# google/neural-light-transport

Hardware: AMD Instinct MI355X
Metric: rendered Mtexels/s at 1024^2 UV (full Model.call forward: U-Net + UV->camera warp); at N > 1: N collective-free replicas of this forward (weak scaling).  The data-parallel TRAIN step with the RCCL gradient all-reduce (BASELINE config 4) is `train_step`: value = Mtexels/s over all ranks, speedup_vs_o (higher is better)
Workload: dtype f32 via 3xbf16 split, 9 exact products, fp32 accumulate (the LDS-tiled encoder convs: fp32 operands as three bf16 terms on v_mfma_f32_16x16x32_bf16, every term product exact in fp32); f32 storage everywhere, every other launch native f32; 1 GPU; BASELINE config 3: dragon_specular relight+view-synth, depth0 16/depth 256, 4 frames/GPU, 1024^2 UV, k=4 obs maps, 512^2 camera warp; frames_per_gpu=4, uv=1024, k=4, cam=512, conv_algo=auto, plan=fused ends, launch=eager, two HIP streams, distinct_batches_rotated=3, launch_tape_replays=0, parallelism=dp1 (frames sharded, no forward collective), world=1, dist_world_size=1, device=cuda:0

## Files before the change

include/nlt_hip.h:

```cpp
#ifndef NLT_HIP_H_
#define NLT_HIP_H_

#ifdef __cplusplus
extern "C" {
#endif

typedef enum {
  NLT_OK = 0,
  NLT_ERR_BAD_ARG = -1,
  NLT_ERR_UNSUPPORTED = -2,
  NLT_ERR_LAUNCH = -3
} nlt_status;

typedef enum {
  NLT_CONV1X1 = 0,
  NLT_CONV_K2S2 = 1,
  NLT_CONV_K2S1 = 2,
  NLT_DECONV_K2S2 = 3,
  NLT_DECONV_K2S1 = 4,
  NLT_CONV_K3S1 = 5,
  NLT_CONV_K3S2 = 6,
  NLT_DECONV_K3S1 = 7,
  NLT_DECONV_K3S2 = 8
} nlt_conv_mode;
// ... 399 lines not shown
                                const float* packed, int cout, int tn, float* out, int ldo,
                                const float* mask_src, int ldm, float mask_alpha, int accumulate, void* stream);

int nlt_conv_c32_supported(int mode, int cin, int cout);
int nlt_conv_c32_forward(int mode, const float* src, int ld, int cin, int frames, int kobs, int h, int w,
                         const float* packed, const float* bias, int cout,
                         float* out, int ldo, float* mean_out, int ldm, int act, float alpha, void* stream);

long nlt_conv_tile_packed_floats(int mode, int cin, int cout, int tn);
int nlt_pack_conv_tile_weights(int mode, const float* w_keras, int cin, int cout, int tn, float* packed, void* stream);
int nlt_conv_tile_forward(int mode, const float* src, int ld, int cin, int frames, int kobs, int h, int w,
                          const float* packed, const float* bias, int cout, int tn,
                          float* out, int ldo, float* mean_out, int ldm, int act, float alpha, void* stream);

int nlt_pack_conv_tile_weights_adjoint(int adj_mode, const float* w_keras, int cpre, int cout, int tn, int full, int lo,
                                       float* packed, void* stream);
int nlt_conv_tile_backward_data(int adj_mode, const float* dpre, int ldp, int cpre, int n, int h, int w,
                                const float* packed, int cout, int tn, float* out, int ldo,
                                const float* mask_src, int ldm, float mask_alpha, int accumulate,
                                int split_c, const float* split_y, float* split_d, float split_alpha, int split_partial,
                                void* stream);

long nlt_conv_tile3_packed_elems(int mode, int cin, int cout, int tn);
int nlt_pack_conv_tile3_weights(int mode, const float* w_keras, int cin, int cout, int tn, unsigned short* packed, void* stream);
int nlt_conv_tile3_forward(int mode, int nprod, const float* src, int ld, int cin, int frames, int kobs, int h, int w,
                           const unsigned short* packed, const float* bias, int cout, int tn,
                           float* out, int ldo, float* mean_out, int ldm, int act, float alpha, void* stream);
int nlt_conv_tile3r_forward(int mode, int nprod, const float* src, int ld, int cin, int frames, int kobs, int h, int w,
                            const unsigned short* packed, const float* bias, int cout, int tn,
                            float* out, int ldo, float* mean_out, int ldm, int act, float alpha, int max_workgroups, void* stream);
int nlt_conv_tile3d_forward(int mode, int nprod, const float* src, int ld, int cin, int frames, int kobs, int h, int w,
                            const unsigned short* packed, const float* bias, int cout, int tn,
                            float* out, int ldo, float* mean_out, int ldm, int act, float alpha, void* stream);
long nlt_conv_tile3w_s2_packed_elems(int cin2, int cout2);
int nlt_pack_conv_tile3w_s2_weights(const float* w_keras, int cin2, int cout2, unsigned short* packed, void* stream);
long nlt_conv_tile3w_s2_lds_bytes(int cin, int cout, int cout2);
int nlt_conv_tile3w_s2_forward(int nprod, const float* src, int ld, int cin, int frames, int kobs, int h, int w,
                               const unsigned short* packed, const float* bias, int cout, float* out, int ldo,
                               float* mean_out, int ldm, int act, float alpha,
                               const unsigned short* packed2, const float* bias2, int cout2, float* out2, int ldo2,
                               int act2, float alpha2, int max_workgroups, void* stream);

long nlt_chmix_bf16_packed_elems(int cin, int cout);
int nlt_chmix_bf16_pack(const float* w_keras, int cin, int cout, unsigned short* packed, void* stream);
int nlt_chmix_bf16_forward(const unsigned short* x, long texels, int cin, const unsigned short* packed,
                           const float* bias, int cout, int act, float alpha, unsigned short* out, void* stream);

int nlt_conv_k3_forward(int mode, int algo, const float* x, int n, int h, int w, int cin,
                        const float* w_keras, const float* bias, int cout, float* y,
                        int act, float alpha, void* stream);

int nlt_conv_k3_backward_data(int mode, int algo, const float* dpre, int n, int h, int w, int cin,
                              const float* w_keras, int cout, float* dx, void* stream);

long nlt_conv_k3_wgrad_workspace_floats(int mode, int n, int h, int w, int cin, int cout);
int nlt_conv_k3_backward_weights(int mode, const float* x, int n, int h, int w, int cin,
                                 const float* dpre, int cout, float* dw_keras, float* dbias,
                                 float* workspace, long workspace_floats, void* stream);

#ifdef __cplusplus
}
#endif
#endif
```

neural-light-transport_amd/_capi.py:

```python
import ctypes
import threading
import os

import torch

_HERE = os.path.dirname(os.path.abspath(__file__))
LIB_PATH = os.environ.get('NLT_HIP_LIB') or os.path.join(_HERE, 'libnlt_hip.so')

CONV1X1, CONV_K2S2, CONV_K2S1, DECONV_K2S2, DECONV_K2S1 = range(5)
CONV_K3S1, CONV_K3S2, DECONV_K3S1, DECONV_K3S2 = range(5, 9)
ALGO_AUTO, ALGO_DIRECT, ALGO_MFMA = range(3)

_c_int, _c_long, _c_float, _vp = ctypes.c_int, ctypes.c_long, ctypes.c_float, ctypes.c_void_p
_c_double = ctypes.c_double
MAP_F64, MAP_F32, MAP_F16 = range(3)

SIGNATURES = {
    'nlt_version': (ctypes.c_char_p, []),
    'nlt_status_string': (ctypes.c_char_p, [_c_int]),
    'nlt_packed_weight_floats': (_c_long, [_c_int] * 4),
    'nlt_pack_conv_weights': (_c_int, [_c_int, _vp, _c_int, _c_int, _c_int, _vp, _vp]),
    'nlt_conv_forward': (_c_int, [_c_int, _c_int, _c_int, _vp, _c_int, _c_int, _vp, _c_int, _c_int,
                                  _c_int, _c_int, _c_int, _vp, _vp, _vp, _c_int, _vp, _c_int,
                                  _c_int, _c_float, _vp, _c_int, _c_int, _vp]),
# ... 83 lines not shown
    'nlt_front_ovr_forward_u8': (_c_int, [_vp] * 4 + [_c_int] * 3 + [_vp] * 5 + [_c_int, _c_float, _vp, _c_int, _vp, _vp, _vp]),
    'nlt_front_obs_forward': (_c_int, [_vp, _vp] + [_c_int] * 3 + [_vp, _vp, _c_float, _c_int] + [_vp] * 3 + [_vp]),
    'nlt_front_obs_forward_u8': (_c_int, [_vp] * 3 + [_c_int] * 3 + [_vp, _vp, _c_float, _c_int] + [_vp] * 3 + [_vp]),
    'nlt_frame_sum_accumulate': (_c_int, [_vp, _c_int, _c_long, _vp, _c_int, _vp]),
    'nlt_frame_mean_finish': (_c_int, [_vp, _c_long, _c_long, _vp, _vp]),
    'nlt_frame_mean_finish_l0': (_c_int, [_vp, _c_long, _c_long, _vp, _vp, _vp, _vp]),
    'nlt_conv_backward_data': (_c_int, [_c_int, _c_int, _c_int, _vp, _vp, _c_int, _c_int, _c_int, _c_int, _c_int, _vp, _vp, _c_int,
                                        _vp, _c_int, _vp, _c_int, _c_float, _c_int, _c_int, _vp, _vp, _c_float, _c_int, _vp]),
    'nlt_conv_tile_packed_floats': (_c_long, [_c_int] * 4),
    'nlt_pack_conv_tile_weights': (_c_int, [_c_int, _vp, _c_int, _c_int, _c_int, _vp, _vp]),
    'nlt_conv_tile_forward': (_c_int, [_c_int, _vp, _c_int, _c_int, _c_int, _c_int, _c_int, _c_int, _vp, _vp, _c_int, _c_int,
                                       _vp, _c_int, _vp, _c_int, _c_int, _c_float, _vp]),
    'nlt_pack_conv_tile_weights_adjoint': (_c_int, [_c_int, _vp, _c_int, _c_int, _c_int, _c_int, _c_int, _vp, _vp]),
    'nlt_conv_c32_supported': (_c_int, [_c_int] * 3),
    'nlt_conv_c32_forward': (_c_int, [_c_int, _vp, _c_int, _c_int, _c_int, _c_int, _c_int, _c_int, _vp, _vp, _c_int,
                                      _vp, _c_int, _vp, _c_int, _c_int, _c_float, _vp]),
    'nlt_conv_wino_packed_floats': (_c_long, [_c_int] * 4),
    'nlt_pack_conv_wino_weights': (_c_int, [_c_int, _vp, _c_int, _c_int, _c_int, _vp, _vp]),
    'nlt_conv_wino_forward': (_c_int, [_c_int, _vp, _c_int, _c_int, _c_int, _c_int, _c_int, _c_int, _vp, _vp, _c_int, _c_int,
                                       _vp, _c_int, _vp, _c_int, _c_int, _c_float, _vp]),
    'nlt_pack_conv_wino_weights_adjoint': (_c_int, [_c_int, _vp, _c_int, _c_int, _c_int, _c_int, _c_int, _vp, _vp]),
    'nlt_conv_wino_backward_data': (_c_int, [_c_int, _vp, _c_int, _c_int, _c_int, _c_int, _c_int, _vp, _c_int, _c_int, _vp, _c_int,
                                             _vp, _c_int, _c_float, _c_int, _vp]),
    'nlt_conv_tile_backward_data': (_c_int, [_c_int, _vp, _c_int, _c_int, _c_int, _c_int, _c_int, _vp, _c_int, _c_int, _vp, _c_int,
                                             _vp, _c_int, _c_float, _c_int, _c_int, _vp, _vp, _c_float, _c_int, _vp]),
    'nlt_conv_tile3_packed_elems': (_c_long, [_c_int] * 4),
    'nlt_pack_conv_tile3_weights': (_c_int, [_c_int, _vp, _c_int, _c_int, _c_int, _vp, _vp]),
    'nlt_conv_tile3_forward': (_c_int, [_c_int, _c_int, _vp, _c_int, _c_int, _c_int, _c_int, _c_int, _c_int, _vp, _vp, _c_int, _c_int,
                                        _vp, _c_int, _vp, _c_int, _c_int, _c_float, _vp]),
    'nlt_conv_tile3r_forward': (_c_int, [_c_int, _c_int, _vp, _c_int, _c_int, _c_int, _c_int, _c_int, _c_int, _vp, _vp, _c_int, _c_int,
                                         _vp, _c_int, _vp, _c_int, _c_int, _c_float, _c_int, _vp]),
    'nlt_conv_tile3d_forward': (_c_int, [_c_int, _c_int, _vp, _c_int, _c_int, _c_int, _c_int, _c_int, _c_int, _vp, _vp, _c_int, _c_int,
                                         _vp, _c_int, _vp, _c_int, _c_int, _c_float, _vp]),
    'nlt_conv_tile3w_s2_packed_elems': (_c_long, [_c_int] * 2),
    'nlt_pack_conv_tile3w_s2_weights': (_c_int, [_vp, _c_int, _c_int, _vp, _vp]),
    'nlt_conv_tile3w_s2_lds_bytes': (_c_long, [_c_int] * 3),
    'nlt_conv_tile3w_s2_forward': (_c_int, [_c_int, _vp, _c_int, _c_int, _c_int, _c_int, _c_int, _c_int, _vp, _vp, _c_int, _vp, _c_int,
                                            _vp, _c_int, _c_int, _c_float, _vp, _vp, _c_int, _vp, _c_int, _c_int, _c_float, _c_int, _vp]),
    'nlt_conv_bf16_packed_elems': (_c_long, [_c_int] * 4),
    'nlt_conv_bf16_pack': (_c_int, [_c_int, _vp, _c_int, _c_int, _c_int, _vp, _vp]),
    'nlt_conv_bf16_forward': (_c_int, [_c_int, _c_int, _vp, _c_int, _c_int, _c_int, _vp, _c_int, _c_int, _c_int,
                                       _c_int, _c_int, _c_int, _vp, _vp, _c_int, _vp, _c_int, _c_int, _c_int, _c_float, _vp]),
    'nlt_conv_bf16_forward_map': (_c_int, [_c_int, _c_int, _vp, _c_int, _c_int, _c_int, _vp, _c_int, _c_int, _c_int,
                                           _c_int, _c_int, _c_int, _vp, _vp, _c_int, _vp, _c_int, _c_int, _c_int, _c_float,
                                           _vp, _c_int, _vp]),
    'nlt_obs_mean_bf16': (_c_int, [_vp, _c_int, _c_int, _c_long, _c_int, _vp, _c_int, _vp]),
    'nlt_chmix_bf16_packed_elems': (_c_long, [_c_int, _c_int]),
    'nlt_chmix_bf16_pack': (_c_int, [_vp, _c_int, _c_int, _vp, _vp]),
    'nlt_chmix_bf16_forward': (_c_int, [_vp, _c_long, _c_int, _vp, _vp, _c_int, _c_int, _c_float, _vp, _vp]),
    'nlt_cosine_map': (_c_int, [_vp] * 4 + [_c_double] * 3 + [_c_long, _vp, _vp, _vp]),
    'nlt_albedo': (_c_int, [_vp, _c_int, _c_long, _vp, _vp, _vp]),
    'nlt_diffuse_base': (_c_int, [_vp, _vp, _c_int, _c_long, _vp, _vp]),
    'nlt_remap_bilinear_u8': (_c_int, [_vp, _c_int, _c_int, _c_int, _vp, _c_int, _c_int, _c_int, _c_int, _c_int, _vp, _vp]),
    'nlt_remap_bilinear_f32': (_c_int, [_vp, _c_int, _c_int, _c_int, _vp, _c_int, _c_int, _c_int, _c_int, _c_int, _vp, _vp]),
    'nlt_capture_camspc': (_c_int, [_vp] * 4 + [_c_double] * 6 + [_vp, _vp, _c_int, _c_int] + [_vp] * 5),
    'nlt_capture_uvspc': (_c_int, [_vp, _c_int, _c_int, _c_int, _vp, _vp, _vp, _c_int, _c_int, _c_int] + [_vp] * 6),
    'nlt_diffuse_bases': (_c_int, [_vp, _vp, _vp] + [_c_int] * 5 + [_vp, _vp, _vp]),
    'nlt_uv_index_map_workspace_bytes': (_c_long, [_c_int, _c_int, _c_long]),
    'nlt_uv_index_map': (_c_int, [_vp, _vp, _c_long, _c_int, _c_int, _c_int, _c_int, _c_double, _vp, _vp, _vp, _vp]),
    'nlt_knn_indices': (_c_int, [_vp, _c_int, _vp, _c_int, _c_int, _vp, _vp]),
    'nlt_psnr_sums': (_c_int, [_vp, _vp, _vp, _c_long, _c_int, _vp, _vp, _vp]),
    'nlt_gather_frames_u8': (_c_int, [_vp, _vp, _c_int, _c_long, _vp, _vp]),
    'nlt_assemble_batch': (_c_int, [_vp] * 6 + [_c_int, _c_int, _c_long, _c_int] + [_vp] * 6 + [_vp]),
    'nlt_warp_backward_det_workspace_bytes': (_c_long, [_c_int] * 5),
    'nlt_warp_backward_det': (_c_int, [_vp, _vp] + [_c_int] * 5 + [_vp, _vp, _c_long, _vp]),
    'nlt_resize_bilinear_backward_gather': (_c_int, [_vp] + [_c_int] * 6 + [_vp, _vp]),
# ... 871 lines not shown

def conv_tile3_forward(mode, src, ld, cin, frames, kobs, h, w, packed, bias, cout, tn, out, ldo, mean_out, ldm,
                       act=True, alpha=0.3, nprod=6):
    _call('nlt_conv_tile3_forward', mode, nprod, _ptr(src), ld, cin, frames, kobs, h, w, packed.data_ptr(), _ptr(bias), cout, tn,
          _ptr(out), ldo, _ptr(mean_out), ldm, 1 if act else 0, float(alpha))


def conv_tile3r_plan(mode, cin, tn):
    if mode not in (CONV_K2S1, CONV_K2S2) or cin % 16 or tn not in (32, 64):
        return None
    if mode == CONV_K2S1 and tn == 32:
        for rows in (4, 2):
            lds = cin * 768 + 8 * 6 * (((rows + 1) * 17 + 15) // 16 * 16) * 16
            if lds <= 160 * 1024:
                return (lds, 8, 1, rows)
    lds = cin * (tn // 16) * 384 + 2 * 6 * (160 if mode == CONV_K2S1 else 272) * 16
    if lds > 160 * 1024:
        return None
    return (lds, 8, 1, 8) if 2 * lds > 160 * 1024 else (lds, 4, 2, 8)


def conv_tile3r_forward(mode, src, ld, cin, frames, kobs, h, w, packed, bias, cout, tn, out, ldo, mean_out, ldm,
                        act=True, alpha=0.3, nprod=6, max_workgroups=0):
    _call('nlt_conv_tile3r_forward', mode, nprod, _ptr(src), ld, cin, frames, kobs, h, w, packed.data_ptr(), _ptr(bias), cout, tn,
          _ptr(out), ldo, _ptr(mean_out), ldm, 1 if act else 0, float(alpha), max_workgroups)


def conv_tile3d_forward(mode, src, ld, cin, frames, kobs, h, w, packed, bias, cout, tn, out, ldo, mean_out, ldm,
                        act=True, alpha=0.3, nprod=6):
    _call('nlt_conv_tile3d_forward', mode, nprod, _ptr(src), ld, cin, frames, kobs, h, w, packed.data_ptr(), _ptr(bias), cout, tn,
          _ptr(out), ldo, _ptr(mean_out), ldm, 1 if act else 0, float(alpha))


def pack_conv_tile3w_s2_weights(w_keras, cin2, cout2):
    return _pack('nlt_conv_tile3w_s2_packed_elems', (cin2, cout2),
                 'nlt_pack_conv_tile3w_s2_weights', (_ptr(_dense(w_keras, 'w_keras')), cin2, cout2), torch.int16, w_keras.device)


def conv_tile3w_s2_plan(cin, cout, cout2):
    n = lib().nlt_conv_tile3w_s2_lds_bytes(cin, cout, cout2)
    return n if n > 0 else None


def conv_tile3w_s2_forward(src, ld, cin, frames, kobs, h, w, packed, bias, cout, mean_out, ldm, packed2, bias2, cout2, out2, ldo2,
                           act=True, alpha=0.3, act2=True, alpha2=0.3, nprod=6, max_workgroups=0, out=None, ldo=0):
    _call('nlt_conv_tile3w_s2_forward', nprod, _ptr(src), ld, cin, frames, kobs, h, w, packed.data_ptr(), _ptr(bias), cout,
          _ptr(out), ldo, _ptr(mean_out), ldm, 1 if act else 0, float(alpha), packed2.data_ptr(), _ptr(bias2), cout2,
          _ptr(out2), ldo2, 1 if act2 else 0, float(alpha2), max_workgroups)


def conv_bf16_pack(mode, w_keras, c0, c1, cout):
    return _pack('nlt_conv_bf16_packed_elems', (mode, c0, c1, cout),
                 'nlt_conv_bf16_pack', (mode, _ptr(_dense(w_keras, 'w_keras')), c0, c1, cout), torch.bfloat16, w_keras.device)


def _any_ptr(t, what):
    if t is None:
        return None, 0
    if not (t.is_cuda and t.dtype in (torch.float32, torch.bfloat16)):
        raise NLTError("%s: expected a float32 / bfloat16 CUDA tensor, got %s on %s" % (what, t.dtype, t.device))
    return t.data_ptr(), 1 if t.dtype == torch.float32 else 0


def conv_bf16_forward(mode, src0, c0, ld0, src1, c1, ld1, n, h, w, w_packed, bias, cout, out, ldo, act=True, alpha=0.3, tile_hint=0):
    p0, f0 = _any_ptr(src0, 'src0')
    p1, f1 = _any_ptr(src1, 'src1')
# ... 367 lines not shown
```

neural-light-transport_amd/csrc/conv_tile3.hip:

```cpp
#include "nlt_common.h"
#include "pack_common.h"

namespace {

typedef __attribute__((ext_vector_type(8))) __bf16 bf16x8;
typedef unsigned short u16;
typedef unsigned int u32x4 __attribute__((ext_vector_type(4)));

constexpr int TH = 8, TW = 16;
constexpr int QS2 = 272, ODD2 = 132;
constexpr int PL = 160;

template <int MODE> struct T3;
template <> struct T3<NLT_CONV_K2S1> { static constexpr int PAIRS = 2, B_UNITS = 153 * 2, B_SLOTS = 6 * PL; };
template <> struct T3<NLT_CONV_K2S2> { static constexpr int PAIRS = 1, B_UNITS = 256 * 2, B_SLOTS = 6 * QS2; };

struct Tile3P {
  const float* src; const u16* packed; const float* bias;
  float* out; float* mean_out;
  int ld, cin, frames, kobs, h, w;
  int oh, ow, cout, ldo, ldm;
  int tiles_y, tiles_x, ncc;
  int act; float alpha;
};
// ... 385 lines not shown
      else load_b(u, ngi, nc, (m + 2 - NM) / KO, (m + 2 - NM) % KO);
      __builtin_amdgcn_sched_barrier(0);
      read_a(lds + a * A_SLOTS, 0, lane, at);
      term_products<NPROD>(at, [&](int t, int rt) { return bt[t][rt]; }, acc[io]);
      if (m == NM - 1 && cc == p.ncc - 1) {
#pragma unroll
        for (int e = 0; e < KO; ++e) epilogue<false>(p, f, gi * KO + e, g * TNT * 16 + 4 * kk, ty0 + wm * RT, tx0 + j, acc[e], mean);
      }
      if (io == KO - 1) {
        store_a(a ^ 1);
        __syncthreads();
      }
    }
    gi = ngi; cc = nc;
  }
}

template <int TNT, int KO>
int launch3d_k(const Tile3P& p, int nprod, hipStream_t s) {
  const dim3 grid((unsigned)((long)p.frames * p.tiles_y * p.tiles_x), (unsigned)(p.cout / (16 * TNT)));
  if (nprod == 9) hipLaunchKernelGGL((conv_tile3d_kernel<TNT, 9, KO>), grid, dim3(256), 0, s, p);
  else hipLaunchKernelGGL((conv_tile3d_kernel<TNT, 6, KO>), grid, dim3(256), 0, s, p);
  NLT_CHECK_LAUNCH();
  return NLT_OK;
}

template <int TNT>
int launch3d(const Tile3P& p, int nprod, hipStream_t s) {
  if (TNT == 2 && p.kobs % 4 == 0) return launch3d_k<TNT, (TNT == 2 ? 4 : 1)>(p, nprod, s);
  if (p.kobs % 2 == 0) return launch3d_k<TNT, 2>(p, nprod, s);
  return launch3d_k<TNT, 1>(p, nprod, s);
}

extern __shared__ u32x4 tile3r_lds[];

template <int MODE, int TNT, int NPROD, int KO, int NWV>
__global__ __launch_bounds__(64 * NWV, 2) void conv_tile3r_kernel(Tile3P p, int ngroups) {
  using TT = T3<MODE>;
  constexpr int NT = 64 * NWV;
  constexpr int WN = TNT == 4 ? 2 : 1, WM = NWV / WN, RT = TH / WM, CT = 2;
  constexpr int A_SLOTS = TT::PAIRS * TNT * 3 * 64;
  constexpr int NB = (TT::B_UNITS + NT - 1) / NT;
  constexpr int BPL = MODE == NLT_CONV_K2S1 ? PL : QS2;
  const int a_group = p.ncc * 2 * TNT * 3 * 64;
  u32x4* const lds_b = tile3r_lds + a_group;

  const int tid = threadIdx.x, lane = tid & 63, wave = tid >> 6;
  const int kk = lane >> 4, j = lane & 15;
  const int wn = wave % WN, wm = wave / WN;
  const int spf = (MODE == NLT_CONV_K2S1 ? 1 : 2) * p.ncc;
  const int groups = p.kobs / KO;
  const long in_frame = (long)p.h * p.w;
  const int tiles = p.frames * p.tiles_y * p.tiles_x;
  const long items = (long)tiles * ngroups;
  const int rank = xcd_tile3(blockIdx.x, gridDim.x);
  int it = (int)(rank * items / gridDim.x);
  const int it_end = (int)((rank + 1) * items / gridDim.x);
  if (it >= it_end) return;

  int b_lds[NB], b_hf[NB]; long b_tex[NB]; bool b_ok[NB], b_st[NB];
#pragma unroll
  for (int i = 0; i < NB; ++i) unit_slot<MODE>(tid + NT * i, b_hf[i], b_lds[i], b_st[i]);
  int ng = 0, nf = 0, nty0 = 0, ntx0 = 0;
  auto geom = [&](int item) {
    ng = item / tiles;
    int t = item - ng * tiles;
// ... 514 lines not shown
    return tn == 64 ? launch3<NLT_CONV_K2S1, 4>(p, nprod, s, resident_wg) : launch3<NLT_CONV_K2S1, 2>(p, nprod, s, resident_wg);
  return tn == 64 ? launch3<NLT_CONV_K2S2, 4>(p, nprod, s, resident_wg) : launch3<NLT_CONV_K2S2, 2>(p, nprod, s, resident_wg);
}

extern "C" int nlt_conv_tile3_forward(int mode, int nprod, const float* src, int ld, int cin, int frames, int kobs, int h, int w,
                                      const unsigned short* packed, const float* bias, int cout, int tn,
                                      float* out, int ldo, float* mean_out, int ldm, int act, float alpha, void* stream) {
  return tile3_forward(mode, nprod, src, ld, cin, frames, kobs, h, w, packed, bias, cout, tn, out, ldo, mean_out, ldm, act, alpha,
                       -1, stream);
}

extern "C" int nlt_conv_tile3r_forward(int mode, int nprod, const float* src, int ld, int cin, int frames, int kobs, int h, int w,
                                       const unsigned short* packed, const float* bias, int cout, int tn,
                                       float* out, int ldo, float* mean_out, int ldm, int act, float alpha, int max_workgroups,
                                       void* stream) {
  if (max_workgroups < 0) return NLT_ERR_BAD_ARG;
  return tile3_forward(mode, nprod, src, ld, cin, frames, kobs, h, w, packed, bias, cout, tn, out, ldo, mean_out, ldm, act, alpha,
                       max_workgroups, stream);
}

extern "C" int nlt_conv_tile3d_forward(int mode, int nprod, const float* src, int ld, int cin, int frames, int kobs, int h, int w,
                                       const unsigned short* packed, const float* bias, int cout, int tn,
                                       float* out, int ldo, float* mean_out, int ldm, int act, float alpha, void* stream) {
  const bool supported = mode == NLT_CONV_K2S2 && nlt_conv_tile3_packed_elems(mode, cin, cout, tn) > 0 && !((h | w) & 1) &&
                         (nprod == 6 || nprod == 9) && !mean_out;
  Tile3P p;
  const int st = tile3_params(p, out != nullptr, supported, true, ldo, true, src, ld, cin, frames, kobs, h, w, packed, bias, cout,
                              out, ldo, mean_out, ldm, act, alpha);
  if (st != NLT_OK) return st;
  hipStream_t s = static_cast<hipStream_t>(stream);
  return tn == 64 ? launch3d<4>(p, nprod, s) : launch3d<2>(p, nprod, s);
}

extern "C" long nlt_conv_tile3w_s2_packed_elems(int cin2, int cout2) {
  return (cin2 == 32 && cout2 == 64) ? (long)12 * cin2 * cout2 : -1;
}

extern "C" int nlt_pack_conv_tile3w_s2_weights(const float* w_keras, int cin2, int cout2, unsigned short* packed, void* stream) {
  const long total = nlt_conv_tile3w_s2_packed_elems(cin2, cout2);
  if (total <= 0) return NLT_ERR_UNSUPPORTED;
  if (!w_keras || !packed || !nlt_aligned16(packed)) return NLT_ERR_BAD_ARG;
  hipLaunchKernelGGL(pack_tile3s2_kernel, dim3((unsigned)((total + 255) / 256)), dim3(256), 0, static_cast<hipStream_t>(stream),
                     w_keras, cin2, cout2, total, packed);
  NLT_CHECK_LAUNCH();
  return NLT_OK;
}

extern "C" long nlt_conv_tile3w_s2_lds_bytes(int cin, int cout, int cout2) {
  return (cin == 32 && cout == 32 && cout2 == 64 && S2_LDS <= TILE3R_LDS_CU) ? (long)S2_LDS : -1;
}

extern "C" int nlt_conv_tile3w_s2_forward(int nprod, const float* src, int ld, int cin, int frames, int kobs, int h, int w,
                                          const unsigned short* packed, const float* bias, int cout, float* out, int ldo,
                                          float* mean_out, int ldm, int act, float alpha,
                                          const unsigned short* packed2, const float* bias2, int cout2, float* out2, int ldo2,
                                          int act2, float alpha2, int max_workgroups, void* stream) {
  const bool own_args = packed2 && bias2 && out2 && max_workgroups >= 0 && cout2 > 0;
  const bool supported = nlt_conv_tile3w_s2_lds_bytes(cin, cout, cout2) > 0 && (nprod == 6 || nprod == 9) && !((h | w) & 1) && !out;
  const bool own_layout = ldo2 >= cout2 && !(ldo2 & 3) && nlt_aligned16(packed2) && nlt_aligned16(bias2) && nlt_aligned16(out2);
  Tile3S2P P;
  const int st = tile3_params(P.a, own_args, supported, own_layout, ldo2, false, src, ld, cin, frames, kobs, h, w, packed, bias, cout,
                              out, ldo, mean_out, ldm, act, alpha);
  if (st != NLT_OK) return st;
  P.packed2 = packed2; P.bias2 = bias2; P.out2 = out2; P.ldo2 = ldo2; P.act2 = act2; P.alpha2 = alpha2;
  return launch3w_s2(P, nprod, max_workgroups, static_cast<hipStream_t>(stream));
}
// ... 1 lines not shown
```

neural-light-transport_amd/engine.py:

```python
import os

import torch

from . import _capi as C
from .engine_infer import OverrideMixin


class OpTimer:

    def __init__(self):
        self.pending, self.records = [], {}
        self.flops = {}
        self.moved = {}

    def launch(self, label, nbytes, fn, *args, **kw):
        e0, e1 = torch.cuda.Event(enable_timing=True), torch.cuda.Event(enable_timing=True)
        e0.record()
        fn(*args, **kw)
        e1.record()
        self.pending.append((label, nbytes, e0, e1))

    def collect(self):
        torch.cuda.synchronize()
        for label, nbytes, e0, e1 in self.pending:
            r = self.records.setdefault(label, [0, 0.0, nbytes])
            r[0] += 1
            r[1] += e0.elapsed_time(e1)
        self.pending = []
        return self.records


def _act_kw(act):
    return {'act': act is not None, 'alpha': act.alpha if act is not None else 0.0}


def _gemm(mode, n, h, w, cin, cout):
    ncols = cout * (4 if mode == C.DECONV_K2S2 else 1)
    taps = 4 if mode in (C.CONV_K2S2, C.CONV_K2S1, C.DECONV_K2S1) else 1
    rows = n * h * w // (4 if mode == C.CONV_K2S2 else 1)
    return rows, ncols, 2 * rows * taps * cin * ncols


CHOICE_DICTS = {'tile': ('tile_hints',), 'direct': ('algo_hints',), 'lds': ('lds_hints',), 'splitk': ('tile_hints', 'splitk_hints'),
                'wino': ('wino_hints',), 'c32': ('c32_hints',)}
HINT_DICTS = tuple(dict.fromkeys(a for attrs in CHOICE_DICTS.values() for a in attrs))
EXCLUSIVE = ('lds', 'wino', 'c32')


def hint_word(hint):
    return hint & 255, bool(hint & 256), bool(hint & 512)


FOLD_S2 = 1024
DIRECT_S2 = 2048
FOLD_HINT = FOLD_S2 + 512 + 32


class RenderPlan(OverrideMixin):
    def __init__(self, net_query, net_obs, use_obs=True):
        self.timer = None
        self.q, self.o, self.use_obs = net_query, net_obs, use_obs
        self.tile_hints = {}
        self.algo_hints = {}
        self.lds_hints = {}
        self.splitk_hints = {}
        self.wino_hints = {}
        self.c32_hints = {}
        self._trial = None
        self._ran = set()
        self.autotune = os.environ.get('NLT_AUTOTUNE', '1') != '0'
        self.fuse_ends = os.environ.get('NLT_FUSED', '1') != '0'
        self._front_blob = None
        self.fuse_override = os.environ.get('NLT_FUSED_OVERRIDE', '1') != '0'
        self._ovr = None
        self.front_l2 = os.environ.get('NLT_FRONT_L2', '1') != '0'
        self.fuse_dec = os.environ.get('NLT_FUSED_DEC', '1') != '0'
        self.front_v4 = os.environ.get('NLT_FRONT4', '1') != '0'
        self.fuse_train = os.environ.get('NLT_FUSED_TRAIN', '1') != '0'
        self.front4_train = os.environ.get('NLT_FRONT4_TRAIN', '1') != '0'
        self.two_streams = os.environ.get('NLT_STREAMS', '2') != '1'
        self._side = None
        self._bside = None
        self.wgrad_tiled = os.environ.get('NLT_WGRAD', 'tiled') != 'atomic'
        self.wgrad_narrow = os.environ.get('NLT_WGRAD_NARROW', '1') != '0'
        self.bwd_streams = int(os.environ.get('NLT_BWD_STREAMS', '1'))
        self.use_tape = os.environ.get('NLT_TAPE', '1') != '0'
        self.fold_split = os.environ.get('NLT_FOLD_SPLIT', '1') != '0'
# ... 99 lines not shown

    def clear_choices(self):
        for a in HINT_DICTS:
            setattr(self, a, {})

    def _tile_splitk(self, label, rows, ncols, star, ok=True):
        kind, hint = self._trial or (None, 0)
        if kind is None:
            tile_hint, ks = self.tile_hints.get(label, self.tile_hints.get('*', 0) if star else 0), self.splitk_hints.get(label, 1)
        else:
            tile_hint, ks = (hint if kind == 'tile' else hint[0] if kind == 'splitk' else 0), 1
        if tile_hint and ((ncols + 15) // 16) % (tile_hint & 15):
            tile_hint = 0
        if kind == 'splitk' and ok:
            rt, ct = (tile_hint >> 4, tile_hint & 15) if tile_hint else (1, 1)
            waves = -(-rows // (16 * rt)) * (-(-ncols // 16) // ct)
            npad = -(-ncols // 16) * 16
            ks = hint[1] if (waves < 4096 and rows * npad * abs(hint[1]) <= (1 << 24)) else 1
        return tile_hint, ks

    def _conv(self, label, layer, act, src0, c0, ld0, src1, c1, ld1, n, h, w, out, ldo, algo=C.ALGO_AUTO, bmap=None):
        layer.build(c0 + c1, src0.device)
        assert layer.cin == c0 + c1, (layer.cin, c0, c1)
        small = (c0 + c1) * layer.n_ch_out <= 1024
        if self._hint('direct', label) == C.ALGO_DIRECT or (self._trying('direct') and small):
            algo = C.ALGO_DIRECT
            self._ran.add((label, 'direct'))
        ok = c0 % 4 == 0 and c1 % 4 == 0 and layer.n_ch_out % 4 == 0 and algo != C.ALGO_DIRECT
        oh, ow = layer.out_hw(h, w)
        nbytes = 4 * (n * h * w * (c0 + c1) + n * oh * ow * layer.n_ch_out)
        rows, ncols, flops = _gemm(layer.mode, n, h, w, c0 + c1, layer.n_ch_out)
        if c1 == 0 and ok and algo == C.ALGO_AUTO and self._wino(label, layer, act, src0, c0, ld0, n, 1, h, w, out, ldo):
            return
        tile_hint, ks = self._tile_splitk(label, rows, ncols, True, ok)
        srcs = (src0, c0, ld0, src1, c1, ld1, n, h, w)
        dst = (layer.bias.detach(), layer.n_ch_out, out, ldo)
        kw = dict(_act_kw(act), flops=flops)
        if bmap is not None:
            if not ok:
                raise C.NLTError("a bias-map conv needs channel counts that are multiples of 4 (%s)" % label)
            if abs(ks) > 1:
                self._ran.add((label, 'splitk'))
            self._launch(label, nbytes, C.conv_forward_map, layer.mode, ks or 1, *srcs, layer.packed(c0, c1), *dst, bmap,
                         tile_hint=tile_hint, w_keras=layer.kernel.detach(), **kw)
        elif abs(ks) > 1 and ok:
            self._ran.add((label, 'splitk'))
            self._launch(label, nbytes, C.conv_forward_splitk, layer.mode, ks, *srcs, layer.packed(c0, c1), *dst,
                         tile_hint=tile_hint, **kw)
        else:
            self._launch(label, nbytes, C.conv_forward, layer.mode, *srcs, layer.kernel.detach(),
                         layer.packed(c0, c1) if ok else None, *dst, algo=algo if ok else C.ALGO_DIRECT,
                         tile_hint=tile_hint if ok else 0, **kw)

    def _mean(self, label, obs, obs_weights, frames, kobs, hw, c, mean_out, ldm):
        self._launch(label.replace('.s1', '.mean'), 4 * frames * hw * c * (kobs + 1), C.obs_mean_forward,
                     obs, obs_weights, frames, kobs, hw, c, mean_out, ldm)

    def _enc_launch(self, fn, packed, extra, kind, unfold, label, layer, act, src, cin, ld, frames, kobs, h, w, out, ldo,
                    mean_out, ldm, **kw):
        oh, ow = layer.out_hw(h, w)
        nf, c = frames * kobs, layer.n_ch_out
        fold_mean = mean_out is not None and not unfold
        nbytes = 4 * (nf * h * w * cin + nf * oh * ow * c)
        if fold_mean:
            nbytes += 4 * frames * oh * ow * c * (kobs + 1)
        self._ran.add((label, kind))
# ... 38 lines not shown
                and nxt.mode == C.CONV_K2S2 and C.conv_tile3w_s2_plan(cin, layer.n_ch_out, nxt.n_ch_out) is not None)

    def _conv_fold(self, label, layer, act, src, cin, ld, frames, kobs, h, w, mean_out, ldm, fold):
        label2, nxt, act2, out2, ldo2 = fold
        nxt.build(layer.n_ch_out, src.device)
        nf, c, c2 = frames * kobs, layer.n_ch_out, nxt.n_ch_out
        nbytes = 4 * (nf * h * w * cin + nf * h * w * c) + 4 * frames * h * w * c * (kobs + 1)
        nbytes += 4 * (nf * h * w * c + nf * (h // 2) * (w // 2) * c2)
        moved = 4 * (nf * h * w * cin + (frames * h * w * c if mean_out is not None else 0) + nf * (h // 2) * (w // 2) * c2)
        self._ran.add((label, 'lds'))
        self._launch(label, nbytes, C.conv_tile3w_s2_forward, src, ld, cin, frames, kobs, h, w, layer.packed_tile3(32),
                     layer.bias.detach(), c, mean_out, ldm, nxt.packed_tile3s2(), nxt.bias.detach(), c2, out2, ldo2,
                     act=act is not None, alpha=act.alpha if act is not None else 0.0,
                     act2=act2 is not None, alpha2=act2.alpha if act2 is not None else 0.0,
                     nprod=9 if self.precision == 'f32x3_9' else 6,
                     flops=2 * nf * h * w * 4 * cin * c + 2 * nf * (h // 2) * (w // 2) * 4 * c * c2, moved=moved)

    def _conv_enc(self, label, layer, act, src, cin, ld, frames, kobs, h, w, out, ldo, algo, mean_out=None, ldm=0,
                  obs_weights=None, fold=None):
        layer.build(cin, src.device)
        conv = (label, layer, act, src, cin, ld, frames, kobs, h, w, out, ldo, mean_out, ldm)
        trial = self._trial is not None
        chint = self._hint('c32', label)
        if (chint and self.use_c32 and algo == C.ALGO_AUTO and obs_weights is None and layer.cin == cin and ld % 4 == 0 and ldo % 4 == 0
                and C.conv_c32_supported(layer.mode, cin, layer.n_ch_out) and not (chint == 2 and kobs == 1 and trial)):
            self._enc_launch(C.conv_c32_forward, layer.packed_tile(32), (), 'c32', chint == 2 and kobs > 1, *conv)
            return
        if (algo == C.ALGO_AUTO and layer.mode == C.CONV_K2S1 and self._hint('wino', label) and self._wino(*conv, obs_weights)):
            return
        hint = self._hint('lds', label)
        tn, unfold, resident = hint_word(hint)
        ok = (tn and obs_weights is None and algo == C.ALGO_AUTO and layer.mode in (C.CONV_K2S2, C.CONV_K2S1)
              and layer.cin == cin and cin % 16 == 0 and layer.n_ch_out % tn == 0)
        if hint & FOLD_S2:
            if ok and fold is not None and hint == FOLD_HINT and ((h | w) & 1) == 0 and self._fold_ok(layer, cin, fold[1]):
                if mean_out is None and kobs == 1:
                    mean_out, ldm = out, ldo
                self._conv_fold(label, layer, act, src, cin, ld, frames, kobs, h, w, mean_out, ldm, fold)
                return True
            ok = ok and not trial
        if ok and resident and (self.precision not in ('f32x3', 'f32x3_9') or C.conv_tile3r_plan(layer.mode, cin, tn) is None):
            ok = not trial
            resident = False
        if ok and unfold and kobs == 1:
            ok = not trial
            unfold = False
        direct = bool(hint & DIRECT_S2)
        if ok and direct and not (self.precision in ('f32x3', 'f32x3_9') and layer.mode == C.CONV_K2S2 and ((h | w) & 1) == 0
                                  and (mean_out is None or unfold)):
            ok = not trial
            direct = False
        if ok and self.precision in ('f32x3', 'f32x3_9'):
            fn = C.conv_tile3d_forward if direct else (C.conv_tile3r_forward if resident else C.conv_tile3_forward)
            self._enc_launch(fn, layer.packed_tile3(tn), (tn,), 'lds', unfold, *conv, nprod=9 if self.precision == 'f32x3_9' else 6)
        elif ok:
            self._enc_launch(C.conv_tile_forward, layer.packed_tile(tn), (tn,), 'lds', unfold, *conv)
        else:
            self._conv(label, layer, act, src, cin, ld, None, 0, 0, frames * kobs, h, w, out, ldo, algo)
            if mean_out is not None:
                oh, ow = layer.out_hw(h, w)
                self._mean(label, out, obs_weights, frames, kobs, oh * ow, layer.n_ch_out, mean_out, ldm)

    def _dec_block_plain(self, b, j, lab, da, dact_a, db, dact_b, srcs, n, hh, ww, algo, s2_label=None, bmap=None):
        nl = da.n_ch_out
        self._conv(s2_label or lab + '.s2', da, dact_a, *srcs, n, hh, ww, b['dtmp'][j], nl, algo, bmap=bmap)
        self._conv(lab + '.s1', db, dact_b, b['dtmp'][j], nl, nl, None, 0, 0, n, 2 * hh, 2 * ww, b['dec'][j], db.n_ch_out, algo)
        return b['dec'][j], db.n_ch_out

    def _autotune(self, run, backward=False):
        saved_timer = self.timer
        self._tuning = True
        results = {}
        trials = [('tile', 16 * r + c) for r in (1, 2, 4) for c in (1, 2, 4)]
        if not self.fuse_ends and not backward:
            trials.append(('direct', 0))
        if not backward:
            trials += [('lds', 32), ('lds', 64), ('lds', 256 + 32), ('lds', 256 + 64)]
            if self.precision in ('f32x3', 'f32x3_9'):
                trials += [('lds', 512 + 32), ('lds', 512 + 64)]
                if self._direct_trial():
                    trials += [('lds', DIRECT_S2 + u + tn) for u in (0, 256) for tn in (32, 64)]
                if self.fold_s2 and self._fold_trial():
                    trials.append(('lds', FOLD_HINT))
        elif self.tile_dgrad:
            trials += [('lds', 32), ('lds', 64)]
        if self.use_c32 and not backward:
            trials += [('c32', 1), ('c32', 2)]
        if self.use_wino:
            trials += [('wino', 32), ('wino', 64)] + ([('wino', 256 + 32), ('wino', 256 + 64)] if not backward else [])
        mode = os.environ.get('NLT_SPLITK', 'all')
        if mode == 'all' or (mode == 'fwd' and not backward):
            forms = os.environ.get('NLT_SPLITK_FORMS', 'both')
            cand = ((4, 8, 16, 32, 64, 128) if forms != 'two' else ()) + ((-16, -32, -64, -128) if forms == 'both' else ()) + \
                   ((-4, -8, -16, -32, -64, -128) if forms == 'two' else ())
            trials += [('splitk', (16 * r + c, ks)) for (r, c) in ((1, 1), (1, 2), (2, 2), (1, 4)) for ks in cand]
        try:
            for kind, hint in trials:
                self._trial, self._ran = (kind, hint), set()
                self.timer = None
                run()
                self.timer = OpTimer()
                run(); run()
                rec = self.timer.collect()
                for label, r in rec.items():
                    t = r[1] / r[0]
                    if label.endswith('.o.s1') and label.replace('.s1', '.mean') in rec:
                        m = rec[label.replace('.s1', '.mean')]
                        t += m[1] / m[0]
                    if kind == 'tile' or (label, kind) in self._ran:
                        results.setdefault(label, []).append((t, kind, hint))
        finally:
            self._trial, self.timer, self._tuning = None, saved_timer, False
        for label, res in results.items():
            t_fold = [t for t, kind, hint in res if kind == 'lds' and hint == FOLD_HINT]
# ... 713 lines not shown
```

neural-light-transport_amd/networks/elements.py:

```python
import math

import torch

from .. import _capi as C

_seed_counter = [0]


def _glorot_uniform(shape, device, seed):
    kh, kw, a, b = shape
    limit = math.sqrt(6.0 / (kh * kw * a + kh * kw * b))
    g = torch.Generator().manual_seed(seed)
    return ((torch.rand(shape, generator=g) * 2 - 1) * limit).to(device)


class Layer:
    built = True
    trainable = ()

    def build(self, cin, device):
        return cin

    def variables(self):
        return []
# ... 97 lines not shown

    def packed_tile(self, tn):
        return self._cached_pack(('tile', tn),
                                 lambda: C.pack_conv_tile_weights(self.mode, self.kernel.detach(), self.cin, self.n_ch_out, tn),
                                 dict(kind=C.REPACK_TILE, mode=self.mode, c0=self.cin, c1=0, cout=self.n_ch_out, tn=tn, lo=0,
                                      full=self.n_ch_out))

    def packed_wino(self, tn):
        return self._cached_pack(('wino', tn),
                                 lambda: C.pack_conv_wino_weights(self.mode, self.kernel.detach(), self.cin, self.n_ch_out, tn),
                                 dict(kind=C.REPACK_WINO, mode=self.mode, c0=self.cin, c1=0, cout=self.n_ch_out, tn=tn, lo=0,
                                      full=self.n_ch_out))

    def packed_adjoint_wino(self, lo, hi, tn):
        adj = self.ADJOINT[self.mode]
        return self._cached_pack(('adjwino', lo, hi, tn),
                                 lambda: C.pack_conv_wino_weights(adj, self.kernel.detach(), self.n_ch_out, hi - lo, tn, self.cin, lo),
                                 dict(kind=C.REPACK_WINO, mode=adj, c0=self.n_ch_out, c1=0, cout=hi - lo, tn=tn, lo=lo, full=self.cin))

    def packed_bf16(self, c0, c1):
        cache = self.__dict__.setdefault('_packed_bf', {})
        ent, ver = cache.get((c0, c1)), self._version()
        if ent is None or ent[0] != ver:
            ent = cache[(c0, c1)] = (ver, C.conv_bf16_pack(self.mode, self.kernel.detach(), c0, c1, self.n_ch_out))
        return ent[1]

    def packed_tile3(self, tn):
        cache = self.__dict__.setdefault('_packed_t3', {})
        ent, ver = cache.get(tn), self._version()
        if ent is None or ent[0] != ver:
            ent = cache[tn] = (ver, C.pack_conv_tile3_weights(self.mode, self.kernel.detach(), self.cin, self.n_ch_out, tn))
        return ent[1]

    def packed_tile3s2(self):
        return self._cached_pack(('tile3s2',), lambda: C.pack_conv_tile3w_s2_weights(self.kernel.detach(), self.cin, self.n_ch_out),
                                 dict(kind=C.REPACK_TILE3S2, mode=self.mode, c0=self.cin, c1=0, cout=self.n_ch_out, tn=0, lo=0,
                                      full=self.n_ch_out))

    ADJOINT = {C.CONV_K2S2: C.DECONV_K2S2, C.CONV_K2S1: C.DECONV_K2S1,
               C.DECONV_K2S2: C.CONV_K2S2, C.DECONV_K2S1: C.CONV_K2S1,
               C.CONV_K3S2: C.DECONV_K3S2, C.CONV_K3S1: C.DECONV_K3S1,
               C.DECONV_K3S2: C.CONV_K3S2, C.DECONV_K3S1: C.CONV_K3S1}

    def packed_adjoint(self, lo, hi):
        k = self.kernel.detach()
        ks = k[..., lo:hi] if self.transpose else k[:, :, lo:hi, :]
        adj = self.ADJOINT[self.mode]
        buf = self._cached_pack(('adj', lo, hi), lambda: C.pack_conv_weights(adj, ks.contiguous(), self.n_ch_out, 0, hi - lo),
                                dict(kind=C.REPACK_MFMA, mode=adj, c0=self.n_ch_out, c1=0, cout=hi - lo, tn=0, lo=lo,
                                     full=self.cin))
        return buf, ks

    def packed_adjoint_tile(self, lo, hi, tn):
        adj = self.ADJOINT[self.mode]
        return self._cached_pack(('adjtile', lo, hi, tn),
                                 lambda: C.pack_conv_tile_weights_adjoint(adj, self.kernel.detach(), self.n_ch_out, hi - lo, tn, self.cin, lo),
                                 dict(kind=C.REPACK_TILE, mode=adj, c0=self.n_ch_out, c1=0, cout=hi - lo, tn=tn, lo=lo, full=self.cin))

    def out_hw(self, h, w):
        if self.mode in (C.CONV_K2S2, C.CONV_K3S2):
            return h // 2, w // 2
        if self.mode in (C.DECONV_K2S2, C.DECONV_K3S2):
            return 2 * h, 2 * w
        return h, w

    def is_plain(self):
# ... 320 lines not shown
```

Before: 3803 Mtexels/s.

## Add LDS-tiled 3xbf16 MFMA kernel for stride-2 transposed convs in decoder

Adds a new tile3t kernel that runs the 2x2 stride-2 transposed convolution (decoder upsampling, with an optional skip-concat second source) as a 3xbf16-split MFMA GEMM. It uses double-buffered LDS weight tiles and scatters the four output taps directly. It comes with a weight packer, C API bindings, and autotune trial hints for 4- or 8-row tiles. The aim is to replace the previous path for these decoder layers with the faster exact-product tiled kernel. The new path is only chosen if the autotuner picks it, and it adds code paths plus packed-weight memory.

```diff
diff --git a/include/nlt_hip.h b/include/nlt_hip.h
--- a/include/nlt_hip.h
+++ b/include/nlt_hip.h
@@ -455,6 +455,14 @@
 int nlt_conv_tile3d_forward(int mode, int nprod, const float* src, int ld, int cin, int frames, int kobs, int h, int w,
                             const unsigned short* packed, const float* bias, int cout, int tn,
                             float* out, int ldo, float* mean_out, int ldm, int act, float alpha, void* stream);
+long nlt_conv_tile3t_packed_elems(int cin, int cout, int tn);
+int nlt_pack_conv_tile3t_weights(const float* w_keras, int cin, int cout, int tn, unsigned short* packed, void* stream);
+int nlt_conv_tile3t_forward(int nprod, const float* src0, int c0, int ld0, const float* src1, int c1, int ld1,
+                            int n, int h, int w, const unsigned short* packed, const float* bias, int cout, int tn,
+                            float* out, int ldo, int act, float alpha, void* stream);
+int nlt_conv_tile3t4_forward(int nprod, const float* src0, int c0, int ld0, const float* src1, int c1, int ld1,
+                             int n, int h, int w, const unsigned short* packed, const float* bias, int cout, int tn,
+                             float* out, int ldo, int act, float alpha, void* stream);
 long nlt_conv_tile3w_s2_packed_elems(int cin2, int cout2);
 int nlt_pack_conv_tile3w_s2_weights(const float* w_keras, int cin2, int cout2, unsigned short* packed, void* stream);
 long nlt_conv_tile3w_s2_lds_bytes(int cin, int cout, int cout2);
diff --git a/neural-light-transport_amd/_capi.py b/neural-light-transport_amd/_capi.py
--- a/neural-light-transport_amd/_capi.py
+++ b/neural-light-transport_amd/_capi.py
@@ -139,6 +139,12 @@
                                          _vp, _c_int, _vp, _c_int, _c_int, _c_float, _c_int, _vp]),
     'nlt_conv_tile3d_forward': (_c_int, [_c_int, _c_int, _vp, _c_int, _c_int, _c_int, _c_int, _c_int, _c_int, _vp, _vp, _c_int, _c_int,
                                          _vp, _c_int, _vp, _c_int, _c_int, _c_float, _vp]),
+    'nlt_conv_tile3t_packed_elems': (_c_long, [_c_int] * 3),
+    'nlt_pack_conv_tile3t_weights': (_c_int, [_vp, _c_int, _c_int, _c_int, _vp, _vp]),
+    'nlt_conv_tile3t_forward': (_c_int, [_c_int, _vp, _c_int, _c_int, _vp, _c_int, _c_int, _c_int, _c_int, _c_int, _vp, _vp, _c_int,
+                                         _c_int, _vp, _c_int, _c_int, _c_float, _vp]),
+    'nlt_conv_tile3t4_forward': (_c_int, [_c_int, _vp, _c_int, _c_int, _vp, _c_int, _c_int, _c_int, _c_int, _c_int, _vp, _vp, _c_int,
+                                          _c_int, _vp, _c_int, _c_int, _c_float, _vp]),
     'nlt_conv_tile3w_s2_packed_elems': (_c_long, [_c_int] * 2),
     'nlt_pack_conv_tile3w_s2_weights': (_c_int, [_vp, _c_int, _c_int, _vp, _vp]),
     'nlt_conv_tile3w_s2_lds_bytes': (_c_long, [_c_int] * 3),
@@ -1076,6 +1082,23 @@
           _ptr(out), ldo, _ptr(mean_out), ldm, 1 if act else 0, float(alpha))
 
 
+def conv_tile3t_supported(c0, c1, cout, tn):
+    return c0 % 32 == 0 and c1 % 32 == 0 and lib().nlt_conv_tile3t_packed_elems(c0 + c1, cout, tn) > 0
+
+
+def pack_conv_tile3t_weights(w_keras, cin, cout, tn):
+    return _pack('nlt_conv_tile3t_packed_elems', (cin, cout, tn),
+                 'nlt_pack_conv_tile3t_weights', (_ptr(_dense(w_keras, 'w_keras')), cin, cout, tn), torch.int16, w_keras.device)
+
+
+def deconv_tile3t_forward(src0, c0, ld0, src1, c1, ld1, n, h, w, packed, bias, cout, tn, out, ldo, act=True, alpha=0.3, nprod=6,
+                        rows=8):
+    if rows not in (4, 8):
+        raise NLTError("deconv_tile3t_forward: rows = %r (4 or 8)" % (rows,))
+    _call('nlt_conv_tile3t_forward' if rows == 8 else 'nlt_conv_tile3t4_forward', nprod, _ptr(src0), c0, ld0, _ptr(src1), c1, ld1,
+          n, h, w, packed.data_ptr(), _ptr(bias), cout, tn, _ptr(out), ldo, 1 if act else 0, float(alpha))
+
+
 def pack_conv_tile3w_s2_weights(w_keras, cin2, cout2):
     return _pack('nlt_conv_tile3w_s2_packed_elems', (cin2, cout2),
                  'nlt_pack_conv_tile3w_s2_weights', (_ptr(_dense(w_keras, 'w_keras')), cin2, cout2), torch.int16, w_keras.device)
diff --git a/neural-light-transport_amd/csrc/conv_tile3.hip b/neural-light-transport_amd/csrc/conv_tile3.hip
--- a/neural-light-transport_amd/csrc/conv_tile3.hip
+++ b/neural-light-transport_amd/csrc/conv_tile3.hip
@@ -441,6 +441,137 @@
   return launch3d_k<TNT, 1>(p, nprod, s);
 }
 
+struct Tile3TP {
+  const float* src0; const float* src1; const u16* packed; const float* bias; float* out;
+  int c0, ld0, ld1, nkb, h, w, cout, ldo;
+  int tiles_y, tiles_x;
+  int act; float alpha;
+};
+
+template <int TNT, int NPROD, int RT>
+__global__ __launch_bounds__(256, 3) void conv_tile3t_kernel(Tile3TP p) {
+  constexpr int CT = TNT;
+  constexpr int A_SLOTS = TNT * 3 * 64;
+  constexpr int NA = (A_SLOTS + 255) / 256;
+  __shared__ u32x4 lds[2 * A_SLOTS];
+
+  const int tid = threadIdx.x, lane = tid & 63, wm = tid >> 6;
+  const int kk = lane >> 4, j = lane & 15;
+  int tile = xcd_tile3(blockIdx.x, gridDim.x);
+  const int tx0 = (tile % p.tiles_x) * TW; tile /= p.tiles_x;
+  const int ty0 = (tile % p.tiles_y) * (4 * RT);
+  const int f = tile / p.tiles_y;
+  const int g = blockIdx.y;
+  const int last = p.nkb - 1;
+
+  int b_off0[RT], b_off1[RT]; bool b_ok[RT];
+#pragma unroll
+  for (int rt = 0; rt < RT; ++rt) {
+    const int y = ty0 + wm * RT + rt, x = tx0 + j;
+    b_ok[rt] = y < p.h && x < p.w;
+    const int tex = b_ok[rt] ? (f * p.h + y) * p.w + x : 0;
+    b_off0[rt] = tex * p.ld0 + 8 * kk;
+    b_off1[rt] = tex * p.ld1 + 8 * kk;
+  }
+
+  u32x4 ra[NA];
+  f32x4 rb[2][RT][2];
+  auto load_a = [&](int q) {
+    const u32x4* ap = reinterpret_cast<const u32x4*>(p.packed) + ((long)g * p.nkb + q) * A_SLOTS;
+#pragma unroll
+    for (int n = 0; n < NA; ++n) ra[n] = ap[(A_SLOTS % 256 == 0 || tid + 256 * n < A_SLOTS) ? tid + 256 * n : tid];
+  };
+  auto store_a = [&](int buf) {
+    u32x4* base = lds + buf * A_SLOTS;
+#pragma unroll
+    for (int n = 0; n < NA; ++n)
+      if (A_SLOTS % 256 == 0 || tid + 256 * n < A_SLOTS) base[tid + 256 * n] = ra[n];
+  };
+  auto load_b = [&](int u, int q) {
+    const int c = 32 * q;
+    const bool second = c >= p.c0;
+    const float* sp = second ? p.src1 + (c - p.c0) : p.src0 + c;
+#pragma unroll
+    for (int rt = 0; rt < RT; ++rt) gather_b_s2(sp + (second ? b_off1[rt] : b_off0[rt]), rb[u][rt][0], rb[u][rt][1]);
+  };
+
+  f32x4 acc[RT][CT];
+#pragma unroll
+  for (int rt = 0; rt < RT; ++rt)
+#pragma unroll
+    for (int ct = 0; ct < CT; ++ct) acc[rt][ct] = (f32x4){0.f, 0.f, 0.f, 0.f};
+
+  load_a(0);
+  load_b(0, 0);
+  load_b(1, last < 1 ? last : 1);
+  store_a(0);
+  __syncthreads();
+  for (int q0 = 0; q0 <= last; q0 += 2) {
+#pragma unroll
+    for (int m = 0; m < 2; ++m) {
+      const int q = q0 + m;
+      if (q <= last) {
+        bf16x8 bt[3][RT], at[3][CT];
+#pragma unroll
+        for (int rt = 0; rt < RT; ++rt) terms_b_s2(b_ok[rt], rb[m][rt][0], rb[m][rt][1], bt[0][rt], bt[1][rt], bt[2][rt]);
+        load_a(q + 1 < last ? q + 1 : last);
+        load_b(m, q + 2 < last ? q + 2 : last);
+        __builtin_amdgcn_sched_barrier(0);
+        read_a(lds + m * A_SLOTS, 0, lane, at);
+        term_products<NPROD>(at, [&](int t, int rt) { return bt[t][rt]; }, acc);
+        store_a(m ^ 1);
+        __syncthreads();
+      }
+    }
+  }
+
+#pragma unroll
+  for (int ct = 0; ct < CT; ++ct) {
+    const int col = (g * TNT + ct) * 16;
+    const int t = col / p.cout, oc = col - t * p.cout + 4 * kk;
+    const f32x4 bv = *reinterpret_cast<const f32x4*>(p.bias + oc);
+#pragma unroll
+    for (int rt = 0; rt < RT; ++rt) {
+      const int y = ty0 + wm * RT + rt, x = tx0 + j;
+      if (b_ok[rt]) {
+        const long ot = ((long)(f * 2 * p.h + 2 * y + (t >> 1)) * (2 * p.w) + 2 * x + (t & 1));
+        *reinterpret_cast<f32x4*>(p.out + ot * p.ldo + oc) = bias_act(acc[rt][ct], bv, p.act, p.alpha);
+      }
+    }
+  }
+}
+
+template <int TNT, int RT>
+int launch3t(const Tile3TP& p, int frames, int nprod, hipStream_t s) {
+  const dim3 grid((unsigned)((long)frames * p.tiles_y * p.tiles_x), (unsigned)(4 * p.cout / (16 * TNT)));
+  if (nprod == 9) hipLaunchKernelGGL((conv_tile3t_kernel<TNT, 9, RT>), grid, dim3(256), 0, s, p);
+  else hipLaunchKernelGGL((conv_tile3t_kernel<TNT, 6, RT>), grid, dim3(256), 0, s, p);
+  NLT_CHECK_LAUNCH();
+  return NLT_OK;
+}
+
+__global__ void pack_tile3t_kernel(const float* __restrict__ wk, int cin, int cout, int tnt, long total, u16* __restrict__ wp) {
+  const long idx = (long)blockIdx.x * blockDim.x + threadIdx.x;
+  if (idx >= total) return;
+  const int e = idx & 7, lane = (idx >> 3) & 63;
+  long r = idx >> 9;
+  const int term = r % 3; r /= 3;
+  const int ct = r % tnt; r /= tnt;
+  const int nkb = cin >> 5;
+  const int q = r % nkb;
+  const int g = r / nkb;
+  const int kk = lane >> 4, i = lane & 15;
+  const int c = q * 32 + kk * 8 + e;
+  const int col = (g * tnt + ct) * 16 + i;
+  const int t = col / cout, o = col % cout;
+  const float v = wk[((long)t * cout + o) * cin + c];
+  const u16 hi = bf16_rne_bits(v);
+  const float r1 = v - bf16_bits_float(hi);
+  const u16 mid = bf16_rne_bits(r1);
+  const float r2 = r1 - bf16_bits_float(mid);
+  wp[idx] = term == 0 ? hi : (term == 1 ? mid : bf16_rne_bits(r2));
+}
+
 extern __shared__ u32x4 tile3r_lds[];
 
 template <int MODE, int TNT, int NPROD, int KO, int NWV>
@@ -1021,6 +1152,55 @@
   return tn == 64 ? launch3d<4>(p, nprod, s) : launch3d<2>(p, nprod, s);
 }
 
+extern "C" long nlt_conv_tile3t_packed_elems(int cin, int cout, int tn) {
+  if (cin <= 0 || cout <= 0 || (cin & 31) || (cout & 15) || (tn != 32 && tn != 64)) return -1;
+  return (long)12 * cin * cout;
+}
+
+extern "C" int nlt_pack_conv_tile3t_weights(const float* w_keras, int cin, int cout, int tn, unsigned short* packed, void* stream) {
+  const long total = nlt_conv_tile3t_packed_elems(cin, cout, tn);
+  if (total <= 0) return NLT_ERR_UNSUPPORTED;
+  if (!w_keras || !packed || !nlt_aligned16(packed)) return NLT_ERR_BAD_ARG;
+  hipLaunchKernelGGL(pack_tile3t_kernel, dim3((unsigned)((total + 255) / 256)), dim3(256), 0, static_cast<hipStream_t>(stream),
+                     w_keras, cin, cout, tn / 16, total, packed);
+  NLT_CHECK_LAUNCH();
+  return NLT_OK;
+}
+
+static int tile3t_forward(int rows, int nprod, const float* src0, int c0, int ld0, const float* src1, int c1, int ld1,
+                          int n, int h, int w, const unsigned short* packed, const float* bias, int cout, int tn,
+                          float* out, int ldo, int act, float alpha, void* stream) {
+  if (!src0 || !packed || !bias || !out || (c1 > 0 && !src1)) return NLT_ERR_BAD_ARG;
+  if (n <= 0 || h <= 0 || w <= 0 || c0 <= 0 || c1 < 0 || cout <= 0) return NLT_ERR_BAD_ARG;
+  if ((c0 & 31) || (c1 & 31) || (cout & 15) || (nprod != 6 && nprod != 9) || (tn != 32 && tn != 64)) return NLT_ERR_UNSUPPORTED;
+  if (ld0 < c0 || (ld0 & 3) || (c1 > 0 && (ld1 < c1 || (ld1 & 3))) || ldo < cout || (ldo & 3)) return NLT_ERR_BAD_ARG;
+  if (!nlt_aligned16(src0) || (c1 > 0 && !nlt_aligned16(src1)) || !nlt_aligned16(packed) || !nlt_aligned16(bias) ||
+      !nlt_aligned16(out)) return NLT_ERR_UNSUPPORTED;
+  const long long texels = (long long)n * h * w;
+  const int ldi = (c1 > 0 && ld1 > ld0) ? ld1 : ld0;
+  if (texels * ldi >= (1ll << 31) || 4 * texels * ldo >= (1ll << 31)) return NLT_ERR_UNSUPPORTED;
+  Tile3TP p;
+  p.src0 = src0; p.src1 = c1 > 0 ? src1 : src0; p.packed = packed; p.bias = bias; p.out = out;
+  p.c0 = c0; p.ld0 = ld0; p.ld1 = c1 > 0 ? ld1 : ld0; p.nkb = (c0 + c1) / 32; p.h = h; p.w = w; p.cout = cout; p.ldo = ldo;
+  p.tiles_y = (h + rows - 1) / rows; p.tiles_x = (w + TW - 1) / TW;
+  p.act = act; p.alpha = alpha;
+  hipStream_t s = static_cast<hipStream_t>(stream);
+  if (rows == 8) return tn == 64 ? launch3t<4, 2>(p, n, nprod, s) : launch3t<2, 2>(p, n, nprod, s);
+  return tn == 64 ? launch3t<4, 1>(p, n, nprod, s) : launch3t<2, 1>(p, n, nprod, s);
+}
+
+extern "C" int nlt_conv_tile3t_forward(int nprod, const float* src0, int c0, int ld0, const float* src1, int c1, int ld1,
+                                       int n, int h, int w, const unsigned short* packed, const float* bias, int cout, int tn,
+                                       float* out, int ldo, int act, float alpha, void* stream) {
+  return tile3t_forward(8, nprod, src0, c0, ld0, src1, c1, ld1, n, h, w, packed, bias, cout, tn, out, ldo, act, alpha, stream);
+}
+
+extern "C" int nlt_conv_tile3t4_forward(int nprod, const float* src0, int c0, int ld0, const float* src1, int c1, int ld1,
+                                        int n, int h, int w, const unsigned short* packed, const float* bias, int cout, int tn,
+                                        float* out, int ldo, int act, float alpha, void* stream) {
+  return tile3t_forward(4, nprod, src0, c0, ld0, src1, c1, ld1, n, h, w, packed, bias, cout, tn, out, ldo, act, alpha, stream);
+}
+
 extern "C" long nlt_conv_tile3w_s2_packed_elems(int cin2, int cout2) {
   return (cin2 == 32 && cout2 == 64) ? (long)12 * cin2 * cout2 : -1;
 }
diff --git a/neural-light-transport_amd/engine.py b/neural-light-transport_amd/engine.py
--- a/neural-light-transport_amd/engine.py
+++ b/neural-light-transport_amd/engine.py
@@ -53,6 +53,8 @@
 
 FOLD_S2 = 1024
 DIRECT_S2 = 2048
+TRANSPOSED_S2 = 4096
+TILE_ROWS4 = 8192
 FOLD_HINT = FOLD_S2 + 512 + 32
 
 
@@ -218,6 +220,15 @@
         rows, ncols, flops = _gemm(layer.mode, n, h, w, c0 + c1, layer.n_ch_out)
         if c1 == 0 and ok and algo == C.ALGO_AUTO and self._wino(label, layer, act, src0, c0, ld0, n, 1, h, w, out, ldo):
             return
+        hint = self._hint('lds', label)
+        if (hint & TRANSPOSED_S2 and self.precision in ('f32x3', 'f32x3_9') and layer.mode == C.DECONV_K2S2 and bmap is None
+                and algo == C.ALGO_AUTO and layer.kernel.is_cuda and ld0 % 4 == 0 and ld1 % 4 == 0 and ldo % 4 == 0
+                and C.conv_tile3t_supported(c0, c1, layer.n_ch_out, hint & 255)):
+            self._ran.add((label, 'lds'))
+            self._launch(label, nbytes, C.deconv_tile3t_forward, src0, c0, ld0, src1, c1, ld1, n, h, w, layer.packed_tile3t(hint & 255),
+                         layer.bias.detach(), layer.n_ch_out, hint & 255, out, ldo, **_act_kw(act),
+                         nprod=9 if self.precision == 'f32x3_9' else 6, rows=4 if hint & TILE_ROWS4 else 8, flops=flops)
+            return
         tile_hint, ks = self._tile_splitk(label, rows, ncols, True, ok)
         srcs = (src0, c0, ld0, src1, c1, ld1, n, h, w)
         dst = (layer.bias.detach(), layer.n_ch_out, out, ldo)
@@ -322,6 +333,8 @@
         tn, unfold, resident = hint_word(hint)
         ok = (tn and obs_weights is None and algo == C.ALGO_AUTO and layer.mode in (C.CONV_K2S2, C.CONV_K2S1)
               and layer.cin == cin and cin % 16 == 0 and layer.n_ch_out % tn == 0)
+        if hint & TRANSPOSED_S2:
+            ok = False
         if hint & FOLD_S2:
             if ok and fold is not None and hint == FOLD_HINT and ((h | w) & 1) == 0 and self._fold_ok(layer, cin, fold[1]):
                 if mean_out is None and kobs == 1:
@@ -370,6 +383,7 @@
                 trials += [('lds', 512 + 32), ('lds', 512 + 64)]
                 if self._direct_trial():
                     trials += [('lds', DIRECT_S2 + u + tn) for u in (0, 256) for tn in (32, 64)]
+                    trials += [('lds', TRANSPOSED_S2 + r + tn) for r in (0, TILE_ROWS4) for tn in (32, 64)]
                 if self.fold_s2 and self._fold_trial():
                     trials.append(('lds', FOLD_HINT))
         elif self.tile_dgrad:
diff --git a/neural-light-transport_amd/networks/elements.py b/neural-light-transport_amd/networks/elements.py
--- a/neural-light-transport_amd/networks/elements.py
+++ b/neural-light-transport_amd/networks/elements.py
@@ -153,6 +153,13 @@
             ent = cache[tn] = (ver, C.pack_conv_tile3_weights(self.mode, self.kernel.detach(), self.cin, self.n_ch_out, tn))
         return ent[1]
 
+    def packed_tile3t(self, tn):
+        cache = self.__dict__.setdefault('_packed_t3t', {})
+        ent, ver = cache.get(tn), self._version()
+        if ent is None or ent[0] != ver:
+            ent = cache[tn] = (ver, C.pack_conv_tile3t_weights(self.kernel.detach(), self.cin, self.n_ch_out, tn))
+        return ent[1]
+
     def packed_tile3s2(self):
         return self._cached_pack(('tile3s2',), lambda: C.pack_conv_tile3w_s2_weights(self.kernel.detach(), self.cin, self.n_ch_out),
                                  dict(kind=C.REPACK_TILE3S2, mode=self.mode, c0=self.cin, c1=0, cout=self.n_ch_out, tn=0, lo=0,
```

Measured after the change: 3711 Mtexels/s. 2.4% lower.
